# IlzeAmandaA/VAE-GP-ODE

Hardware: AMD Instinct MI355X
Metric: latent_trajectories_per_sec (higher is better)
Workload: dtype f32; 1 GPU; configs[1]: ode1 DF q=6 M=100 S=256 T=16 batch=256; step = full ELBO training step (encoder, GP draw, rk4 rollout, decoder, ELBO, backward, Adam), L=1; global_batch=256, mc_draws=1, solver=rk4 (3/8 rule), parallelism=dp1, hip_graph=True, graph_scope=whole, gp_side_stream=True, batchnorm=per-process statistics

## Files before the change

include/gpode.h:

```cpp
#ifndef GPODE_H
#define GPODE_H
#include <stddef.h>
#ifdef __cplusplus
extern "C" {
#endif

#define GPODE_KERNEL_RBF 0
#define GPODE_KERNEL_DF 1
#define GPODE_METHOD_EULER 0
#define GPODE_METHOD_RK4 1
#define GPODE_METHOD_MIDPOINT 2
#define GPODE_METHOD_DOPRI5 3

const char* gpode_version(void);
const char* gpode_last_error(void);
const char* gpode_last_launch(void);
int gpode_supported(int kernel, int Di, int Do);

int gpode_cache_sizes(int kernel, int Di, int Do, int M, int S, size_t* pack_floats, size_t* ws_floats);

int gpode_cache_build_fwd(int kernel, int Di, int Do, int M, int S,
                          const float* raw_ell, const float* raw_var, const float* Z,
                          const float* Um, const float* Us_packed,
                          const float* eps_u, const float* rff_w, const float* rff_eps, const float* rff_u,
                          float* pack, float* ws,
                          float* ell, float* var, float* omega, float* phase, float* u,
                          float* Lu, float* nu, float* u_prior, void* stream);

int gpode_rhs_fwd(int kernel, int Di, int Do, int M, int S, const float* pack,
                  const float* x, int N, float* f, int mode, void* stream);

int gpode_rollout_fwd(int kernel, int order, int method, int Di, int Do, int M, int S,
                      const float* pack, const float* z0, const float* ts, int N, int T,
                      float* zt, float* xstage, void* stream);

int gpode_rollout_bwd(int kernel, int order, int method, int Di, int Do, int M, int S,
                      const float* pack, const float* xstage, const float* gzt, const float* ts, int N, int T,
                      float* gz0, float* astage, void* stream);

int gpode_rhs_vjp(int kernel, int Di, int Do, int M, int S, const float* pack,
                  const float* x, const float* a, int R, float* gx, void* stream);

int gpode_param_grad(int kernel, int Di, int Do, int M, int S, const float* pack,
                     const float* x, const float* a, int R, float* slab, int nchunk, float* gpack, int accumulate,
                     void* stream);

int gpode_cache_bwd_sizes(int kernel, int Di, int Do, int M, int S, size_t* bws_floats);
int gpode_cache_build_bwd(int kernel, int Di, int Do, int M, int S,
                          const float* raw_ell, const float* raw_var, const float* Z, const float* eps_u,
// ... 284 lines not shown
```

vae-gp-ode_amd/_lib.py:

```python
import ctypes
import os

_HERE = os.path.dirname(os.path.abspath(__file__))
LIB_PATH = os.path.join(_HERE, 'libgpode_hip.so')

_vp = ctypes.c_void_p
_i = ctypes.c_int
_f = ctypes.c_float
_sz = ctypes.c_size_t
_sz_p = ctypes.POINTER(_sz)

SIGNATURES = {
    'gpode_version': (ctypes.c_char_p, []),
    'gpode_last_error': (ctypes.c_char_p, []),
    'gpode_last_launch': (ctypes.c_char_p, []),
    'gpode_supported': (_i, [_i, _i, _i]),
    'gpode_cache_sizes': (_i, [_i, _i, _i, _i, _i, _sz_p, _sz_p]),
    'gpode_cache_build_fwd': (_i, [_i] * 5 + [_vp] * 20),
    'gpode_cache_bwd_sizes': (_i, [_i, _i, _i, _i, _i, _sz_p]),
    'gpode_cache_build_bwd': (_i, [_i] * 5 + [_vp] * 13 + [_i, _vp]),
    'gpode_cache_bwd_prepare': (_i, [_i] * 5 + [_vp] * 2 + [_vp]),
    'gpode_cache_info': (_i, [_vp, ctypes.POINTER(_i), _vp]),
    'gpode_cache_pivots': (_i, [_vp, ctypes.POINTER(_f), _vp]),
    'gpode_set_backward_solves': (_i, [_i]),
    'gpode_kernel_matrix': (_i, [_i, _i, _i, _vp, _vp, _vp, _i, _vp, _i, _vp, _vp]),
    'gpode_conditional_ws': (_i, [_i, _i, _i, _i, _sz_p]),
    'gpode_conditional': (_i, [_i, _i, _i, _i] + [_vp] * 5 + [_i, _vp, _i] + [_vp] * 3 + [_vp]),
    'gpode_conditional_df_ws': (_i, [_i, _i, _i, _sz_p]),
    'gpode_conditional_df': (_i, [_i, _i, _i] + [_vp] * 6 + [_i] + [_vp] * 3 + [_vp]),
    'gpode_svgp_kl_fwd': (_i, [_i, _i, _vp, _vp, _vp, _vp]),
    'gpode_svgp_kl_bwd': (_i, [_i, _i] + [_vp] * 5 + [_vp]),
    'gpode_rhs_fwd': (_i, [_i] * 5 + [_vp, _vp, _i, _vp, _i, _vp]),
    'gpode_rollout_fwd': (_i, [_i] * 7 + [_vp, _vp, _vp, _i, _i, _vp, _vp, _vp]),
    'gpode_rollout_bwd': (_i, [_i] * 7 + [_vp] * 4 + [_i, _i, _vp, _vp, _vp]),
    'gpode_rhs_vjp': (_i, [_i] * 5 + [_vp, _vp, _vp, _i, _vp, _vp]),
    'gpode_rhs_jvp': (_i, [_i] * 6 + [_vp, _vp, _i, _vp, _i, _i, _vp, _vp, _i, _vp]),
    'gpode_rollout_jvp': (_i, [_i] * 8 + [_vp, _vp, _i, _vp, _i, _vp, _i, _i, _i, _i, _vp, _vp, _vp]),
    'gpode_param_grad': (_i, [_i] * 5 + [_vp, _vp, _vp, _i, _vp, _i, _vp, _i, _vp]),
    'gpode_cache_sizes_n': (_i, [_i] * 6 + [_sz_p, _sz_p]),
    'gpode_cache_build_fwd_n': (_i, [_i] * 6 + [_vp] * 20),
    'gpode_rollout_fwd_n': (_i, [_i] * 8 + [_vp, _vp, _vp, _i, _i, _vp, _vp, _vp]),
    'gpode_rollout_bwd_n': (_i, [_i] * 8 + [_vp] * 4 + [_i, _i, _vp, _vp, _vp]),
    'gpode_rollout_adaptive_fwd_n': (_i, [_i] * 8 + [_vp] * 3 + [_i, _i, _f, _f, _i] + [_vp] * 5 + [_vp]),
    'gpode_rollout_adaptive_bwd_n': (_i, [_i] * 8 + [_vp] * 5 + [_i, _i, _i, _vp, _vp, _vp]),
    'gpode_rollout_dense_fwd_n': (_i, [_i] * 8 + [_vp] * 3 + [_i, _i, _f, _f, _i] + [_vp] * 6 + [_vp]),
    'gpode_rollout_dense_bwd_n': (_i, [_i] * 8 + [_vp] * 6 + [_i, _i, _i, _vp, _vp, _vp]),
    'gpode_rollout_fwd_nz': (_i, [_i] * 8 + [_vp, _vp, _vp, _i, _i, _vp, _vp, _i, _vp]),
    'gpode_rollout_adaptive_fwd_nz': (_i, [_i] * 8 + [_vp] * 3 + [_i, _i, _f, _f, _i] + [_vp] * 5 + [_i, _vp]),
# ... 132 lines not shown
```

vae-gp-ode_amd/csrc/capi.hip:

```cpp
#include "../../include/gpode.h"
#include "gp_launch.hpp"

namespace gp {
char* error_slot() {
  static thread_local char buf[512] = {0};
  return buf;
}
const char** last_launch_slot() {
  static thread_local const char* tag = "";
  return &tag;
}
bool* force_substep_kernels() {
  static bool on = false;
  return &on;
}
}

extern "C" {

const char* gpode_version(void) { return "gpode-hip 0.1 (gfx950)"; }
const char* gpode_last_error(void) { return gp::error_slot(); }
const char* gpode_last_launch(void) { return *gp::last_launch_slot(); }
int gpode_supported(int kernel, int Di, int Do) { return gp::dims_supported(kernel, Di, Do); }

int gpode_cache_sizes(int kernel, int Di, int Do, int M, int S, size_t* pack_floats, size_t* ws_floats) {
  return gp::cache_sizes(kernel, Di, Do, M, S, pack_floats, ws_floats, 1);
}
int gpode_cache_sizes_n(int kernel, int Di, int Do, int M, int S, int ndraws, size_t* pack_floats, size_t* ws_floats) {
  return gp::cache_sizes(kernel, Di, Do, M, S, pack_floats, ws_floats, ndraws);
}

int gpode_cache_build_fwd_n(int kernel, int Di, int Do, int M, int S, int ndraws,
                            const float* raw_ell, const float* raw_var, const float* Z,
                            const float* Um, const float* Us_packed,
                            const float* eps_u, const float* rff_w, const float* rff_eps, const float* rff_u,
                            float* pack, float* ws,
                            float* ell, float* var, float* omega, float* phase, float* u,
                            float* Lu, float* nu, float* u_prior, void* stream) {
  if (!raw_ell || !raw_var || !Z || !Um || !Us_packed || !eps_u || !rff_w || !rff_eps || !rff_u || !pack || !ws)
    return gp::set_error("gpode_cache_build_fwd: null required pointer");
  return gp::cache_build_fwd(kernel, Di, Do, M, S, ndraws, raw_ell, raw_var, Z, Um, Us_packed, eps_u, rff_w, rff_eps, rff_u,
                             pack, ws, ell, var, omega, phase, u, Lu, nu, u_prior, (hipStream_t)stream);
}
int gpode_cache_build_fwd(int kernel, int Di, int Do, int M, int S,
                          const float* raw_ell, const float* raw_var, const float* Z,
                          const float* Um, const float* Us_packed,
                          const float* eps_u, const float* rff_w, const float* rff_eps, const float* rff_u,
                          float* pack, float* ws,
                          float* ell, float* var, float* omega, float* phase, float* u,
                          float* Lu, float* nu, float* u_prior, void* stream) {
  return gpode_cache_build_fwd_n(kernel, Di, Do, M, S, 1, raw_ell, raw_var, Z, Um, Us_packed, eps_u, rff_w, rff_eps, rff_u, pack, ws, ell, var,
                                 omega, phase, u, Lu, nu, u_prior, stream);
}

int gpode_cache_info(const float* ws, int* host_info, void* stream) {
// ... 867 lines not shown
```

vae-gp-ode_amd/csrc/conv_fwd_v2.hpp:

```cpp
#pragma once
#include "conv_mfma.hpp"

namespace gp {

template <class L> struct FwV2 {
  using PL = FwdPolicy<L, L::CO>;
  template <int CLS> using C = typename PL::template C<CLS>;
  static constexpr int KC = L::CI, NC = L::CO, KK = L::K * L::K, KG = KC / 4;
  static_assert(NC == 16 && L::S == 2 && PL::NCLS == 4, "one co tile, four stride-parity classes");
  static constexpr int NKS = KK * KG;
  static constexpr int NPX = C<0>::npc;
  static_assert(C<1>::npc == NPX && C<2>::npc == NPX && C<3>::npc == NPX && C<1>::nx == C<0>::nx && C<2>::nx == C<0>::nx &&
                C<3>::nx == C<0>::nx, "the classes share one q-grid");
  static constexpr int SH = L::HI, OHW = L::HO * L::HO;
  static constexpr int SRC = KC * SH * SH;
  static constexpr int PS = PL::PS, HP = PL::HP, PADL = PL::PADL, IMG = KC * PS;
  static constexpr int NCW = 4, NTHR = 64 * (NCW + 4), NLT = NTHR - 64 * NCW;
  static constexpr int TPW = 2;
  static constexpr int WIN = 16 * NCW * TPW;
  static constexpr int PF = 2;
  static constexpr int NBUF = (2 * WIN - 2) / NPX + 2;
  static constexpr int MAXS = PADL * (HP + 1);
  static constexpr int TFO = (HP * HP + 3) / 4 * 4;
  static_assert(igemm_tf_in_pad<PL>(), "the input-transform table fits the plane tails");
// ... 205 lines not shown
            }
          }
        });
      }
      __syncthreads();
    }
  }

  if constexpr (STATS) {
    float* red = s_buf + E::RED;
    float* s_sm = red + E::NSW * 2 * NC;
    const int lr = lane & 15, lk = lane >> 4;
#pragma unroll
    for (int e = 0; e < 2; ++e)
#pragma unroll
      for (int r = 0; r < 4; ++r) {
        const float a = row_allreduce16(bs[e][r]), b = row_allreduce16(bq[e][r]);
        if (lr == 0 && wave >= NCW) {
          red[((wave - NCW + NCW * e) * NC + 4 * lk + r) * 2] = a;
          red[((wave - NCW + NCW * e) * NC + 4 * lk + r) * 2 + 1] = b;
        }
      }
    __syncthreads();
    if (tid < 2 * NC) {
      float t = 0.f;
      for (int wv = 0; wv < E::NSW; ++wv) t += red[wv * 2 * NC + tid];
      s_sm[tid] = t;
    }
    __syncthreads();
    bn_sink_publish<NC, E::NTHR>(sink, s_sm);
  }
}

}
```

vae-gp-ode_amd/csrc/conv_mfma.hpp:

```cpp
#pragma once
#include <hip/hip_runtime.h>
#include <cstdint>
#include <type_traits>
#include "bn_math.hpp"
#include "bn_sink.hpp"

namespace gp {

typedef float f32x4 __attribute__((ext_vector_type(4)));

template <int N, class F> __device__ __forceinline__ void static_for(F&& f) {
  if constexpr (N > 0) {
    static_for<N - 1>(f);
    f(std::integral_constant<int, N - 1>{});
  }
}

#ifdef CONVT_PROBE
__device__ unsigned long long g_probe[8];
#define PROBE_T(v) const long long v = clock64()
#define PROBE_ADD(i, v) do { if (threadIdx.x == 0 && blockIdx.x == 0) g_probe[i] += (unsigned long long)(clock64() - (v)); } while (0)
#else
#define PROBE_T(v)
#define PROBE_ADD(i, v)
// ... 75 lines not shown
    const float* wp = sw + ((size_t)t * KC + cb + lk) * WROW + lr;
    const int ao = CG::tap_off(t) + cb * PS;
#pragma unroll
    for (int kk = 0; kk < KB; ++kk) {
#pragma unroll
      for (int c = 0; c < NCJ; ++c) bf[kk][c] = wp[4 * kk * WROW + c * 16];
#pragma unroll
      for (int g = 0; g < NG; ++g) af[kk][g] = s_img[abase[g] + ao + 4 * kk * PS];
    }
  };
  auto mma = [&](const float (&bf)[KB][NCJ], const float (&af)[KB][NG]) {
#pragma unroll
    for (int kk = 0; kk < KB; ++kk)
#pragma unroll
      for (int g = 0; g < NG; ++g)
#pragma unroll
        for (int c = 0; c < NCJ; ++c)
          acc[g][c] = __builtin_amdgcn_mfma_f32_16x16x4f32(bf[kk][c], af[kk][g], acc[g][c], 0, 0, 0);
  };
  fetch(0, bfA, afA);
  int s = 0;
  while (true) {
    if (s + 1 < nsteps) fetch(s + 1, bfB, afB);
    mma(bfA, afA);
    if (++s >= nsteps) break;
    if (s + 1 < nsteps) fetch(s + 1, bfA, afA);
    mma(bfB, afB);
    if (++s >= nsteps) break;
  }
}

extern __shared__ __attribute__((aligned(16))) float igemm_smem[];

template <class PL, int IPB, int TG, int NCJ, bool PAIR, int NTHR, bool STATS = false>
__global__ __launch_bounds__(NTHR, NTHR == 256 ? 2 : 1) void k_conv_igemm(const float* __restrict__ x, const float* __restrict__ w,
                                                      const float* __restrict__ bias, float* __restrict__ y, int B,
                                                      const float* __restrict__ in_bn, BnSink sink) {
  constexpr int KC = PL::KC, NC = PL::NC, NCS = PL::NCS, NCLS = PL::NCLS, SH = PL::SH, OH = PL::OH, HP = PL::HP, PS = PL::PS;
  constexpr int PADL = PL::PADL, WROW = PL::WROW, NWE = PL::NWE;
  static_assert(NCS % 16 == 0 && NC % NCS == 0 && KC % 4 == 0 && NTHR % 256 == 0, "MFMA tiling");
  constexpr int NW = NTHR / 64;
  constexpr int PT = NTHR;
  constexpr int NCO = NCS / 16;
  static_assert(NCO % NCJ == 0, "channel tiles per job");
  constexpr int NJ = NCO / NCJ;
  static_assert(NJ == 1 || TG == 1, "tile groups share all channel tiles");
  static_assert(!STATS || NJ == 1, "output statistics: a lane keeps the same channels in every job of a pass");
  constexpr int IMG = KC * PS;
  static_assert(IMG % 4 == 0, "float4 zero fill");
  constexpr int SRC = KC * SH * SH;
  static_assert(SRC % 4 == 0, "float4 source fetch");
  constexpr int NLD = (IPB * SRC / 4 + PT - 1) / PT;
  float* s_img = igemm_smem;
  float* s_w = igemm_smem + IPB * IMG;
  constexpr int TFO = (HP * HP + 3) / 4 * 4;
  constexpr bool TF_PAD = igemm_tf_in_pad<PL>();
  float* s_sm = s_w + PL::WSLAB + (TF_PAD ? 0 : 4 * KC);
  float4* s_tf_tail = reinterpret_cast<float4*>(s_w + PL::WSLAB);
  auto tf_slot = [&](int ch) -> float4* { return TF_PAD ? reinterpret_cast<float4*>(s_img + ch * PS + TFO) : s_tf_tail + ch; };
  const int tid = threadIdx.x, lane = tid & 63, wave = __builtin_amdgcn_readfirstlane(tid >> 6);
  const int lr = lane & 15, lk = lane >> 4;
  const int ptid = tid;
  const int ngroups = (B + IPB - 1) / IPB;
  const float4* x4 = reinterpret_cast<const float4*>(x);
  const int jw = (wave & 3) * (NW / 4) + (wave >> 2);

  PROBE_T(pt_all);
  for (int e = tid; e < IPB * IMG / 4; e += NTHR) reinterpret_cast<float4*>(s_img)[e] = float4{0.f, 0.f, 0.f, 0.f};
  if (in_bn) {
    if (TF_PAD) __syncthreads();
    for (int e = tid; e < KC; e += NTHR) *tf_slot(e) = reinterpret_cast<const float4*>(in_bn)[e];
  }
  if (STATS)
    for (int e = tid; e < 2 * NC; e += NTHR) s_sm[e] = 0.f;

  constexpr int NPASS = NC / NCS;
  const bool spread = NPASS > 1 && gridDim.x % NPASS == 0;
  const int gstride = spread ? gridDim.x / NPASS : gridDim.x;
  const int gfirst = spread ? blockIdx.x % gstride : blockIdx.x;
  for (int pass = spread ? blockIdx.x / gstride : 0; pass < (spread ? blockIdx.x / gstride + 1 : NPASS); ++pass) {
    const int n0 = pass * NCS;
    __syncthreads();
    PROBE_T(pt_w);
    for (int base = 0; base < NWE; base += NTHR * 8) {
      float v[8];
#pragma unroll
      for (int u = 0; u < 8; ++u) {
        const int e = base + tid + NTHR * u;
        v[u] = e < NWE ? w[PL::w_src(e, n0)] : 0.f;
      }
#pragma unroll
      for (int u = 0; u < 8; ++u) {
        const int e = base + tid + NTHR * u;
        if (e < NWE) s_w[PL::w_dst(e)] = v[u];
      }
    }
    PROBE_ADD(0, pt_w);

    float kshift[NCJ][4], bs[NCJ][4], bq[NCJ][4];
#pragma unroll
    for (int cc = 0; cc < NCJ; ++cc)
#pragma unroll
      for (int r = 0; r < 4; ++r) {
        kshift[cc][r] = STATS ? bn_sink_shift(sink, n0 + cc * 16 + 4 * lk + r) : 0.f;
        bs[cc][r] = bq[cc][r] = 0.f;
      }
    float4 pre[NLD];
    auto prefetch = [&](int grp) __attribute__((always_inline)) {
      const int b0 = grp * IPB;
      const int nf4 = min(IPB, B - b0) * (SRC / 4);
      const float4* src = x4 + (size_t)b0 * (SRC / 4);
#pragma unroll
      for (int i = 0; i < NLD; ++i) {
        const int f = ptid + PT * i;
        if (f < nf4) pre[i] = src[f];
      }
// ... 18 lines not shown
    };
    auto jobs = [&](const float* __restrict__ img, int b0, int nimg, int pf_grp) {
      PROBE_T(pt_rng);
      int wtot = 0;
      constexpr int NCG = PAIR ? NCLS / 2 : NCLS;
      static_for<NCG>([&](auto c) {
        constexpr int c0 = PAIR ? 2 * decltype(c)::value : decltype(c)::value;
        using G0 = typename PL::template C<c0>;
        using G1 = typename PL::template C<PAIR ? c0 + 1 : c0>;
        wtot += ((nimg * G0::npc + 15) / 16) * NJ * (G0::ntaps + (PAIR ? G1::ntaps : 0));
      });
      const int lo = (wtot * jw) / NW, hi = (wtot * (jw + 1)) / NW;
      int cbase = 0;
      PROBE_ADD(0, pt_rng);
      static_for<NCG>([&](auto c) {
        constexpr int c0 = PAIR ? 2 * decltype(c)::value : decltype(c)::value;
        using G = typename PL::template C<c0>;
        using G1 = typename PL::template C<PAIR ? c0 + 1 : c0>;
        static_assert(!PAIR || (G::npc == G1::npc && G::nx == G1::nx), "paired classes cover the same pixel grid");
        static_assert(!PAIR || (G::out_off(0) == G1::out_off(0) + 1 && G::out_off(G::npc - 1) == G1::out_off(G::npc - 1) + 1 &&
                                G1::out_off(0) % 2 == 0 && OH % 2 == 0), "paired classes write neighbouring, 8-byte aligned columns");
        constexpr int ntaps = G::ntaps + (PAIR ? G1::ntaps : 0), npc = G::npc;
        const float* swc = s_w + G::slab_taps * KC * WROW;
        const float* swc1 = s_w + G1::slab_taps * KC * WROW;
        const int mtot = nimg * npc;
        const int njobs = ((mtot + 15) / 16) * NJ;
        const int nlo = lo - cbase - ntaps / 2, nhi = hi - cbase - ntaps / 2;
        const int ub = min(njobs, nlo <= 0 ? 0 : (nlo + ntaps - 1) / ntaps), ue = min(njobs, nhi <= 0 ? 0 : (nhi + ntaps - 1) / ntaps);
        cbase += njobs * ntaps;
        for (int u0 = ub; u0 < ue; u0 += TG) {
          PROBE_T(pt_su);
          const int ng = min(TG, ue - u0);
          const int t0 = u0 / NJ, jc = u0 % NJ;
          int abase[TG], abase1[TG];
#pragma unroll
          for (int g = 0; g < TG; ++g) {
            int m = (t0 + g) * 16 + lr;
            m = (g < ng && m < mtot) ? m : 0;
            const int im = m / npc, p = m % npc;
            abase[g] = im * IMG + lk * PS + G::pix_addr(p);
            abase1[g] = im * IMG + lk * PS + G1::pix_addr(p);
          }
          f32x4 acc[TG][NCJ], acc1[TG][NCJ];
#pragma unroll
          for (int g = 0; g < TG; ++g)
#pragma unroll
            for (int cc = 0; cc < NCJ; ++cc) acc[g][cc] = acc1[g][cc] = f32x4{0.f, 0.f, 0.f, 0.f};
          float bv[NCJ][4];
#pragma unroll
          for (int cc = 0; cc < NCJ; ++cc)
#pragma unroll
            for (int r = 0; r < 4; ++r) bv[cc][r] = bias ? bias[n0 + (jc * NCJ + cc) * 16 + 4 * lk + r] : 0.f;
          PROBE_ADD(6, pt_su);
          PROBE_T(pt_mm);
          auto run = [&](auto gtag, const float* sw, const int (&ab)[TG], f32x4 (&ac)[TG][NCJ]) {
            using GG = typename decltype(gtag)::type;
            switch (ng) {
              case 1: igemm_tile_mma<GG, 1, TG, NCJ, KC, WROW, PS>(img, sw, ab, lk, lr, ac); break;
              case 2: if constexpr (TG >= 2) igemm_tile_mma<GG, 2, TG, NCJ, KC, WROW, PS>(img, sw, ab, lk, lr, ac); break;
              case 3: if constexpr (TG >= 3) igemm_tile_mma<GG, 3, TG, NCJ, KC, WROW, PS>(img, sw, ab, lk, lr, ac); break;
              default: if constexpr (TG >= 4) igemm_tile_mma<GG, 4, TG, NCJ, KC, WROW, PS>(img, sw, ab, lk, lr, ac); break;
            }
          };
          run(std::common_type<G>{}, swc + jc * NCJ * 16, abase, acc);
          if (pf_grp >= 0) { prefetch(pf_grp); pf_grp = -1; }
          if constexpr (PAIR) run(std::common_type<G1>{}, swc1 + jc * NCJ * 16, abase1, acc1);
          PROBE_ADD(3, pt_mm);
          PROBE_T(pt_st);
#pragma unroll
          for (int g = 0; g < TG; ++g) {
            const int m = (t0 + g) * 16 + lr;
            if (g < ng && m < mtot) {
              const int im = m / npc, p = m % npc;
              const int ch0 = n0 + jc * NCJ * 16 + 4 * lk;
              float* yp = y + ((size_t)(b0 + im) * NC + ch0) * (OH * OH) + (PAIR ? G1::out_off(p) : G::out_off(p));
#pragma unroll
              for (int cc = 0; cc < NCJ; ++cc)
#pragma unroll
                for (int r = 0; r < 4; ++r) {
                  const float v0 = acc[g][cc][r] + bv[cc][r];
                  if constexpr (PAIR) {
                    const float v1 = acc1[g][cc][r] + bv[cc][r];
                    *reinterpret_cast<float2*>(yp + (size_t)(cc * 16 + r) * (OH * OH)) = float2{v1, v0};
                    if (STATS) { const float d = v1 - kshift[cc][r]; bs[cc][r] += d; bq[cc][r] = fmaf(d, d, bq[cc][r]); }
                  } else {
                    yp[(size_t)(cc * 16 + r) * (OH * OH)] = v0;
                  }
                  if (STATS) { const float d = v0 - kshift[cc][r]; bs[cc][r] += d; bq[cc][r] = fmaf(d, d, bq[cc][r]); }
                }
            }
          }
          PROBE_ADD(4, pt_st);
        }
      });
      if (pf_grp >= 0) prefetch(pf_grp);
    };
    if (gfirst < ngroups) prefetch(gfirst);
    for (int grp = gfirst; grp < ngroups; grp += gstride) {
      const int b0 = grp * IPB;
      const int nimg = min(IPB, B - b0);
      PROBE_T(pt_b1);
      __syncthreads();
      PROBE_ADD(1, pt_b1);
      PROBE_T(pt_sc);
      scatter(s_img, nimg);
      __syncthreads();
      PROBE_ADD(2, pt_sc);
      PROBE_T(pt_pf);
      PROBE_ADD(7, pt_pf);
      jobs(s_img, b0, nimg, grp + gstride < ngroups ? grp + gstride : -1);
    }
    if constexpr (STATS) {
      __syncthreads();
      float* red = s_w;
#pragma unroll
      for (int cc = 0; cc < NCJ; ++cc)
#pragma unroll
        for (int r = 0; r < 4; ++r) {
          const float a = row_allreduce16(bs[cc][r]), b = row_allreduce16(bq[cc][r]);
          if (lr == 0 && wave < NW) {
            red[(wave * NCS + cc * 16 + 4 * lk + r) * 2] = a;
            red[(wave * NCS + cc * 16 + 4 * lk + r) * 2 + 1] = b;
          }
        }
      __syncthreads();
      if (tid < 2 * NCS) {
        float t = 0.f;
        for (int wv = 0; wv < NW; ++wv) t += red[wv * NCS * 2 + tid];
        s_sm[2 * n0 + tid] = t;
      }
    }
  }
  if constexpr (STATS) {
// ... 226 lines not shown
```

vae-gp-ode_amd/csrc/gp_launch.hpp:

```cpp
#pragma once
#include <cstdint>
#include <cstdlib>
#include <hip/hip_runtime.h>
#include <cstdarg>
#include <cstdio>
#include <mutex>
#include <unordered_map>

namespace gp {

char* error_slot();
const char** last_launch_slot();

inline int set_error(const char* fmt, ...) {
  va_list ap;
  va_start(ap, fmt);
  vsnprintf(error_slot(), 512, fmt, ap);
  va_end(ap);
  return 1;
}

inline int check_launch(const char* what) {
  *last_launch_slot() = what;
  hipError_t e = hipGetLastError();
  if (e != hipSuccess) return set_error("%s: launch failed: %s", what, hipGetErrorString(e));
  return 0;
}

inline bool env_flag(const char* name) {
  const char* e = getenv(name);
  return e && e[0] == '1';
}

template <class... T> inline bool aligned16(const T*... p) {
  return ((uintptr_t{0} | ... | reinterpret_cast<uintptr_t>(p)) & 15) == 0;
}

inline int set_max_lds(const void* kern, size_t bytes) {
  if (bytes <= 64 * 1024) return 0;
  static std::mutex mu;
  static std::unordered_map<const void*, size_t> done;
  std::lock_guard<std::mutex> lock(mu);
  auto it = done.find(kern);
  if (it != done.end() && it->second >= bytes) return 0;
  hipError_t e = hipFuncSetAttribute(kern, hipFuncAttributeMaxDynamicSharedMemorySize, (int)bytes);
  if (e != hipSuccess) return set_error("hipFuncSetAttribute(max dynamic LDS=%zu): %s", bytes, hipGetErrorString(e));
  done[kern] = bytes;
  return 0;
}

inline int ew_grid(size_t n) { size_t g = (n + 255) / 256; return (int)(g < 8192 ? (g ? g : 1) : 8192); }

inline int num_cus() {
  static const int n = [] {
    int dev = 0, v = 0;
    if (hipGetDevice(&dev) != hipSuccess || hipDeviceGetAttribute(&v, hipDeviceAttributeMultiprocessorCount, dev) != hipSuccess || v <= 0)
// ... 207 lines not shown
```

vae-gp-ode_amd/csrc/vae_conv_tiled.hip:

```cpp
#include <hip/hip_runtime.h>
#include <cstdlib>
#include "gp_launch.hpp"
#include "conv_layers.hpp"
#include "conv_mfma.hpp"
#include "conv_dec10_mfma.hpp"
#include "conv_dec1_mfma.hpp"
#include "conv_dec4_mfma.hpp"

namespace gp {

extern __shared__ __attribute__((aligned(16))) float tsm[];

template <class L, int IPB>
__global__ __launch_bounds__(256) void k_convT_fwd(const float* __restrict__ x, const float* __restrict__ w,
                                                    const float* __restrict__ bias, float* __restrict__ y, int B) {
  constexpr int CI = L::CI, CO = L::CO, HI = L::HI, HO = L::HO, HP = L::HP, K = L::K, S = L::S, P = L::P, PL = L::PL;
  constexpr int CPT = CO % 16 == 0 ? 16 : 8;
  static_assert(CO % CPT == 0, "8 or 16 output channels per thread");
  constexpr int NG = CO / CPT;
  constexpr int IMG = CI * HP * HP;
  float* s_img = tsm;
  float* s_w = tsm + IPB * IMG;
  const int tid = threadIdx.x;
  const int b0 = blockIdx.x * IPB;
// ... 275 lines not shown
  }
}

__global__ void k_sum_splits_t(const float* __restrict__ part, int nsplit, size_t n, float* __restrict__ out) {
  const size_t e = (size_t)blockIdx.x * blockDim.x + threadIdx.x;
  if (e >= n) return;
  float acc = 0.f;
  for (int s = 0; s < nsplit; ++s) acc += part[(size_t)s * n + e];
  out[e] = acc;
}

template <class L> static bool matches(const ConvGeom& g) {
  return g.Ci == L::CO && g.Co == L::CI && g.H == L::HO && g.Ho == L::HI && g.K == L::K && g.S == L::S && g.P == L::P;
}

static bool use_mfma() {
  static const bool valu = env_flag("GPODE_CONV_VALU");
  return !valu;
}

constexpr int kSinkMaxWg = 512;

template <class PL, int IPB, int TG, int NCJ, bool PAIR = false, int NTHR = 512, bool STATS = false>
static int launch_igemm(const float* x, const float* w, const float* bias, float* y, int B, hipStream_t st, const char* what,
                        const float* in_bn = nullptr, const BnSink* sink = nullptr) {
  constexpr size_t lds = igemm_lds_bytes<PL, IPB, STATS>();
  static_assert(lds <= (NTHR >= 512 ? 160 : 80) * 1024, "LDS budget");
  auto km = k_conv_igemm<PL, IPB, TG, NCJ, PAIR, NTHR, STATS>;
  if (set_max_lds((const void*)km, lds)) return 1;
  const int ngroups = (B + IPB - 1) / IPB;
  const int cap = num_cus() * (NTHR >= 512 ? 1 : 2);
  if (STATS && cap > kSinkMaxWg) return set_error("%s: more workgroups than the statistics scratch holds", what);
  hipLaunchKernelGGL(km, ngroups < cap ? ngroups : cap, NTHR, lds, st, x, w, bias, y, B, in_bn, STATS ? *sink : BnSink{});
  return check_launch(what);
}

template <class L, int IPB, int IPBM, int COS>
static int launch_T1(const float* x, const float* w, const float* bias, float* y, int B, hipStream_t st, const float* in_bn,
                     const BnSink* sink = nullptr) {
  if (use_mfma() && aligned16(x, w, y, in_bn)) {
    constexpr int TG = COS >= 64 ? 1 : (COS >= 32 ? 2 : 4);
    constexpr bool PAIR = L::S == 2 && (L::HO % 2 == 0) && (L::P % 2 == 1);
    if (sink) return launch_igemm<FwdPolicy<L, COS>, IPBM, TG, COS / 16, PAIR, 512, true>(x, w, bias, y, B, st, "convT_fwd_mfma_stats", in_bn, sink);
    return launch_igemm<FwdPolicy<L, COS>, IPBM, TG, COS / 16, PAIR>(x, w, bias, y, B, st, "convT_fwd_mfma", in_bn);
  }
  if (sink) return set_error("convT forward with output statistics needs the matrix-core path (16-byte aligned operands, GPODE_CONV_VALU unset)");
  if (in_bn) return set_error("convT forward with a fused BatchNorm input needs the matrix-core path (16-byte aligned operands, GPODE_CONV_VALU unset)");
  constexpr int MAXTAPS = ((L::K + L::S - 1) / L::S) * ((L::K + L::S - 1) / L::S);
  const size_t lds = sizeof(float) * ((size_t)IPB * L::CI * L::HP * L::HP + (size_t)MAXTAPS * L::CI * L::CO);
  auto kern = k_convT_fwd<L, IPB>;
  if (set_max_lds((const void*)kern, lds)) return 1;
  hipLaunchKernelGGL(kern, (B + IPB - 1) / IPB, 256, lds, st, x, w, bias, y, B);
  return check_launch("convT_fwd_tiled");
}

template <class L, int IPB, int COC>
static int launch_T2(const float* gy, const float* w, float* gx, int B, hipStream_t st) {
  const size_t lds = sizeof(float) * ((size_t)IPB * L::CO * L::GP_ * L::GP_ + (size_t)COC * L::K * L::K * L::CI);
  auto kern = k_convT_bwd_data<L, IPB, COC>;
  if (set_max_lds((const void*)kern, lds)) return 1;
  hipLaunchKernelGGL(kern, (B + IPB - 1) / IPB, 256, lds, st, gy, w, gx, B);
  return check_launch("convT_bwd_data_tiled");
}

template <class L, int WM, int WN, int WT>
static int launch_wgrad_mfma(const float* x, const float* gy, float* gw, float* scratch, int B, hipStream_t st, const float* in_bn) {
  constexpr int IPBM = 8, NTHR = WM * WN * WT * 64;
// ... 5 lines not shown
  const int ngroups = (B + IPBM - 1) / IPBM;
  const int nwg = ngroups < num_cus() ? ngroups : num_cus();
  if (in_bn) hipLaunchKernelGGL(kb, nwg, NTHR, ldsm, st, x, gy, scratch, B, in_bn);
  else hipLaunchKernelGGL(km, nwg, NTHR, ldsm, st, x, gy, scratch, B, in_bn);
  const size_t n = (size_t)L::CI * L::CO * L::K * L::K;
  if (reduce_job(RedJob{scratch, gw, nwg, (int)n, 1, L::CI / 16, L::CO / 16, L::K * L::K}, st)) return 1;
  return check_launch("convT_wgrad_mfma");
}

template <class L, int COW>
static int launch_T3(const float* x, const float* gy, float* gw, float* scratch, int B, hipStream_t st, const float* in_bn) {
  if (in_bn) return set_error("convT weight gradient with a fused BatchNorm input needs the matrix-core path (16-byte aligned operands, GPODE_CONV_VALU unset)");
  constexpr int NT = L::CI * (COW / 4), PSPLIT = 256 / NT, KK = L::K * L::K;
  size_t fl = (size_t)L::HI * L::HI * L::CI + (size_t)L::GP_ * L::GP_ * COW;
  const size_t red = PSPLIT > 1 ? (size_t)PSPLIT * NT * KK * 4 : 0;
  if (red > fl) fl = red;
  const size_t lds = sizeof(float) * fl;
  int nsplit = B < 256 ? B : 256;
  const int bps = (B + nsplit - 1) / nsplit;
  nsplit = (B + bps - 1) / bps;
  auto kern = k_convT_wgrad<L, COW>;
  if (set_max_lds((const void*)kern, lds)) return 1;
  hipLaunchKernelGGL(kern, dim3(nsplit, L::CO / COW), 256, lds, st, x, gy, scratch, B, bps);
  const size_t n = (size_t)L::CI * L::CO * KK;
  if (reduce_job(RedJob{scratch, gw, nsplit, (int)n, 0, 0, 0, 0}, st)) return 1;
  return check_launch("convT_wgrad_tiled");
}


int conv_v2_dec7_bwd_data(const float* gy, const float* w, float* gx, int B, hipStream_t st);
int conv_v2_dec4_bwd_data(const float* gy, const float* w, float* gx, int B, hipStream_t st);
int conv_v2_dec7_fwd(const float* x, const float* w, const float* bias, float* y, int B, const float* in_bn, const BnSink* sink,
                     hipStream_t st);
static bool conv_v1() {
  static const bool on = env_flag("GPODE_CONV_V1");
  return on;
}

int tiled_bwd_data(const float* gy, const float* w, const float* bias, float* gx, const ConvGeom& g, const float* in_bn, hipStream_t st,
                   const BnSink* sink) {
  if (g.H != g.W || g.Ho != g.Wo) return -1;
  const int B = g.B;
  if (sink && !(matches<Dec7>(g) || matches<Dec4>(g) ||
                (matches<Dec1>(g) && !in_bn)))
    return set_error("gpode_convT_fwd_stats: no specialisation for this geometry");
  const bool mfma = use_mfma() && aligned16(gy, w, gx, in_bn);
  if (matches<Dec7>(g)) {
    if (mfma && !conv_v1()) return conv_v2_dec7_fwd(gy, w, bias, gx, B, in_bn, sink, st);
    return launch_T1<Dec7, 3, 2, 16>(gy, w, bias, gx, B, st, in_bn, sink);
  }
  if (matches<Dec4>(g)) {
    static const int tapcols = [] { const char* e = getenv("GPODE_DEC4_TAPCOLS"); return e ? (e[0] == '1' ? 1 : 0) : -1; }();
    if ((tapcols == 1 || (tapcols < 0 && B <= 4 * num_cus())) && mfma) {
      const size_t lds = sizeof(float) * (dec4::NPI * dec4::TLD + 4 * dec4::CI + (sink ? 2 * dec4::CO * dec4::NPO : 0));
      if (set_max_lds((const void*)dec4::k_fwd<true>, lds) || set_max_lds((const void*)dec4::k_fwd<false>, lds) ||
          set_max_lds((const void*)dec4::k_fwd<true, true>, lds) || set_max_lds((const void*)dec4::k_fwd<false, true>, lds)) return 1;
      const int nwg = B < num_cus() ? B : num_cus();
      const BnSink sk = sink ? *sink : BnSink{};
      if (sink && in_bn) hipLaunchKernelGGL((dec4::k_fwd<true, true>), nwg, 512, lds, st, gy, w, bias, gx, B, in_bn, sk);
      else if (sink) hipLaunchKernelGGL((dec4::k_fwd<false, true>), nwg, 512, lds, st, gy, w, bias, gx, B, in_bn, sk);
      else if (in_bn) hipLaunchKernelGGL((dec4::k_fwd<true>), nwg, 512, lds, st, gy, w, bias, gx, B, in_bn, sk);
      else hipLaunchKernelGGL((dec4::k_fwd<false>), nwg, 512, lds, st, gy, w, bias, gx, B, in_bn, sk);
      return check_launch("dec4_fwd_tapcols");
    }
    return launch_T1<Dec4, 3, 2, 16>(gy, w, bias, gx, B, st, in_bn, sink);
  }
  if (matches<Dec1>(g)) {
    if (!in_bn && mfma) {
      const size_t lds = sizeof(float) * 2 * dec1::NPI * dec1::TLD;
      if (set_max_lds((const void*)dec1::k_fwd<false>, lds) || set_max_lds((const void*)dec1::k_fwd<true>, lds)) return 1;
      const int cap = 2 * num_cus();
      if (sink) hipLaunchKernelGGL(dec1::k_fwd<true>, B < cap ? B : cap, 256, lds, st, gy, w, bias, gx, B, *sink);
      else hipLaunchKernelGGL(dec1::k_fwd<false>, B < cap ? B : cap, 256, lds, st, gy, w, bias, gx, B, BnSink{});
      return check_launch("dec1_fwd_mfma");
    }
    if (sink) return set_error("convT forward with output statistics needs the matrix-core path (16-byte aligned operands, GPODE_CONV_VALU unset)");
    return launch_T1<Dec1, 8, 8, 64>(gy, w, bias, gx, B, st, in_bn);
  }
  if (matches<Enc3>(g) && !in_bn && B >= 96) {
    constexpr int IPB = 2;
    constexpr int MAXTAPS = ((Enc3::K + Enc3::S - 1) / Enc3::S) * ((Enc3::K + Enc3::S - 1) / Enc3::S);
    const size_t lds = sizeof(float) * ((size_t)IPB * Enc3::CI * Enc3::HP * Enc3::HP + (size_t)MAXTAPS * Enc3::CI * Enc3::CO);
    auto kern = k_convT_fwd<Enc3, IPB>;
    if (set_max_lds((const void*)kern, lds)) return 1;
    hipLaunchKernelGGL(kern, (B + IPB - 1) / IPB, 256, lds, st, gy, w, bias, gx, B);
    return check_launch("enc_conv3_bwd_data_tiled");
  }
  if (matches<Enc6>(g) && mfma) {
    if (B < 4 * num_cus()) return launch_igemm<FwdPolicy<Enc6, 16>, 2, 4, 1>(gy, w, bias, gx, B, st, "enc_conv6_bwd_data_mfma", in_bn);
    return launch_igemm<FwdPolicy<Enc6, 16>, 8, 4, 1>(gy, w, bias, gx, B, st, "enc_conv6_bwd_data_mfma", in_bn);
  }
  if (matches<Dec10>(g)) {
    if (mfma) {
      const size_t ldsm = sizeof(float) * dec10::KK * dec10::PST;
      if (set_max_lds((const void*)dec10::k_fwd<true>, ldsm) || set_max_lds((const void*)dec10::k_fwd<false>, ldsm)) return 1;
      if (in_bn) hipLaunchKernelGGL(dec10::k_fwd<true>, B < num_cus() ? B : num_cus(), 512, ldsm, st, gy, w, bias, gx, B, in_bn);
// ... 220 lines not shown
```

vae-gp-ode_amd/csrc/vae_conv_v2.hip:

```cpp
#include <hip/hip_runtime.h>
#include <cstdint>
#include "gp_launch.hpp"
#include "conv_layers.hpp"
#include "conv_bwd_v2.hpp"
#include "conv_fwd_v2.hpp"

namespace gp {

template <class L> static int launch_bwd_data_v2(const float* gy, const float* w, float* gx, int B, hipStream_t st, const char* what) {
  using E = BdV2<L>;
  constexpr size_t lds = E::lds_bytes();
  static_assert(lds <= 160 * 1024, "LDS budget");
  auto km = k_conv_bwd_data_v2<L>;
  if (set_max_lds((const void*)km, lds)) return 1;
  hipLaunchKernelGGL(km, B < num_cus() ? B : num_cus(), E::NTHR, lds, st, gy, w, gx, B);
  return check_launch(what);
}

int conv_v2_dec7_bwd_data(const float* gy, const float* w, float* gx, int B, hipStream_t st) {
  return launch_bwd_data_v2<Dec7>(gy, w, gx, B, st, "conv_v2_dec7_bwd_data");
}

int conv_v2_dec4_bwd_data(const float* gy, const float* w, float* gx, int B, hipStream_t st) {
  return launch_bwd_data_v2<Dec4>(gy, w, gx, B, st, "conv_v2_dec4_bwd_data");
}

template <class L, bool HAS_BN, bool STATS>
static int launch_fwd_v2(const float* x, const float* w, const float* bias, float* y, int B, const float* in_bn, const BnSink* sink,
                         hipStream_t st, const char* what) {
  using E = FwV2<L>;
  constexpr size_t lds = E::lds_bytes(STATS);
  static_assert(lds + (STATS ? sizeof(float) * (E::NTHR + 1) : 0) <= 160 * 1024, "LDS budget (with bn_sink_publish's static arrays)");
  auto km = k_conv_fwd_v2<L, HAS_BN, STATS>;
  if (set_max_lds((const void*)km, lds)) return 1;
  if (STATS && num_cus() > 512) return set_error("%s: more workgroups than the statistics scratch holds", what);
  const int nwork = STATS ? (B + E::IPG - 1) / E::IPG : B;
  hipLaunchKernelGGL(km, nwork < num_cus() ? nwork : num_cus(), E::NTHR, lds, st, x, w, bias, y, B, in_bn, STATS ? *sink : BnSink{});
  return check_launch(what);
}

int conv_v2_dec7_fwd(const float* x, const float* w, const float* bias, float* y, int B, const float* in_bn, const BnSink* sink,
                     hipStream_t st) {
  if (in_bn && sink) return launch_fwd_v2<Dec7, true, true>(x, w, bias, y, B, in_bn, sink, st, "conv_v2_dec7_fwd_bn_stats");
  if (sink) return launch_fwd_v2<Dec7, false, true>(x, w, bias, y, B, in_bn, sink, st, "conv_v2_dec7_fwd_stats");
  if (in_bn) return launch_fwd_v2<Dec7, true, false>(x, w, bias, y, B, in_bn, sink, st, "conv_v2_dec7_fwd_bn");
  return launch_fwd_v2<Dec7, false, false>(x, w, bias, y, B, in_bn, sink, st, "conv_v2_dec7_fwd");
}

}
```

Baseline: 110,200 trajectories/s.

## Add warp-specialized MFMA forward kernel for Dec4 transposed conv with stats read-back

Result: no change. 109,600 trajectories/s (-0.5%).

```diff
diff --git a/include/gpode.h b/include/gpode.h
--- a/include/gpode.h
+++ b/include/gpode.h
@@ -15,6 +15,7 @@
 const char* gpode_version(void);
 const char* gpode_last_error(void);
 const char* gpode_last_launch(void);
+const char* gpode_last_launch_engine(void);
 int gpode_supported(int kernel, int Di, int Do);
 
 int gpode_cache_sizes(int kernel, int Di, int Do, int M, int S, size_t* pack_floats, size_t* ws_floats);
diff --git a/vae-gp-ode_amd/_lib.py b/vae-gp-ode_amd/_lib.py
--- a/vae-gp-ode_amd/_lib.py
+++ b/vae-gp-ode_amd/_lib.py
@@ -14,6 +14,7 @@
     'gpode_version': (ctypes.c_char_p, []),
     'gpode_last_error': (ctypes.c_char_p, []),
     'gpode_last_launch': (ctypes.c_char_p, []),
+    'gpode_last_launch_engine': (ctypes.c_char_p, []),
     'gpode_supported': (_i, [_i, _i, _i]),
     'gpode_cache_sizes': (_i, [_i, _i, _i, _i, _i, _sz_p, _sz_p]),
     'gpode_cache_build_fwd': (_i, [_i] * 5 + [_vp] * 20),
diff --git a/vae-gp-ode_amd/csrc/capi.hip b/vae-gp-ode_amd/csrc/capi.hip
--- a/vae-gp-ode_amd/csrc/capi.hip
+++ b/vae-gp-ode_amd/csrc/capi.hip
@@ -10,6 +10,10 @@
   static thread_local const char* tag = "";
   return &tag;
 }
+const char** last_engine_slot() {
+  static thread_local const char* engine = "";
+  return &engine;
+}
 bool* force_substep_kernels() {
   static bool on = false;
   return &on;
@@ -21,6 +25,7 @@
 const char* gpode_version(void) { return "gpode-hip 0.1 (gfx950)"; }
 const char* gpode_last_error(void) { return gp::error_slot(); }
 const char* gpode_last_launch(void) { return *gp::last_launch_slot(); }
+const char* gpode_last_launch_engine(void) { return *gp::last_engine_slot(); }
 int gpode_supported(int kernel, int Di, int Do) { return gp::dims_supported(kernel, Di, Do); }
 
 int gpode_cache_sizes(int kernel, int Di, int Do, int M, int S, size_t* pack_floats, size_t* ws_floats) {
diff --git a/vae-gp-ode_amd/csrc/conv_fwd_v2.hpp b/vae-gp-ode_amd/csrc/conv_fwd_v2.hpp
--- a/vae-gp-ode_amd/csrc/conv_fwd_v2.hpp
+++ b/vae-gp-ode_amd/csrc/conv_fwd_v2.hpp
@@ -261,4 +261,170 @@
   }
 }
 
+template <class L> struct FwV2P {
+  using PL = FwdPolicy<L, 16>;
+  template <int CLS> using C = typename PL::template C<CLS>;
+  static constexpr int KC = L::CI, NC = L::CO, KK = L::K * L::K, KG = KC / 4, NCT = NC / 16;
+  static_assert(L::S == 2 && PL::NCLS == 4 && NC % 16 == 0 && KC % 4 == 0, "four stride-parity classes, whole MFMA tiles");
+  static constexpr int SH = L::HI, SQ = SH * SH, OHW = L::HO * L::HO;
+  static constexpr int SRC = KC * SQ;
+  static constexpr int PS = PL::PS, HP = PL::HP, PADL = PL::PADL, IMG = KC * PS;
+  static constexpr int NCW = 4, NTHR = 64 * (NCW + 4), NLT = NTHR - 64 * NCW;
+  static constexpr int TSPLIT = NCW / NCT;
+  static constexpr int TPW = 2;
+  static constexpr int WIN = 16 * TSPLIT * TPW;
+  static constexpr int PF = 2;
+  static constexpr int NPMIN = C<0>::npc;
+  static_assert(C<1>::npc >= NPMIN && C<2>::npc >= NPMIN && C<3>::npc >= NPMIN && C<3>::npc < 256, "ring sized for class 0; position in 8 bits");
+  static constexpr int NBUF = (2 * WIN - 2) / NPMIN + 2;
+  static constexpr int MAXW = C<0>::ntaps * KG;
+  static_assert(C<1>::ntaps <= C<0>::ntaps && C<2>::ntaps <= C<0>::ntaps && C<3>::ntaps <= C<0>::ntaps && MAXW <= 160, "weights of a phase in registers");
+  static constexpr int MAXS = PADL * (HP + 1);
+  static constexpr int TFO = (HP * HP + 3) / 4 * 4;
+  static_assert(igemm_tf_in_pad<PL>(), "the input-transform table fits the plane tails");
+  static_assert(NCW % NCT == 0 && TPW * (PF + 1) <= 15, "consumers split the co tiles evenly; LDS reads in flight within what lgkmcnt counts");
+  static constexpr int NSUB = NLT / SQ, NLD = (KG + NSUB - 1) / NSUB;
+  static_assert(SRC % 4 == 0 && NSUB >= 1, "float4 source, producer offset table");
+  static_assert(4 * (MAXS + (KG - 1) * 4 * PS) < 65536, "operand offsets fit the ds_read immediate");
+  static constexpr int CST = NBUF * IMG;
+  static constexpr size_t lds_bytes() { return sizeof(float) * ((size_t)CST + NC); }
+};
+
+template <class E, class G>
+__device__ __forceinline__ void fwv2p_tiles(const float* __restrict__ s_buf, const int (&base)[E::TPW], const float (&wr)[G::ntaps * E::KG],
+                                            f32x4 (&acc)[E::TPW]) {
+  constexpr int N = G::ntaps * E::KG;
+  float bf[E::PF + 1][E::TPW];
+  auto fetch = [&](auto sc) {
+    constexpr int S = decltype(sc)::value;
+    const int off = E::MAXS + G::tap_off(S / E::KG) + (S % E::KG) * 4 * E::PS;
+#pragma unroll
+    for (int t = 0; t < E::TPW; ++t) bf[S % (E::PF + 1)][t] = s_buf[base[t] + off];
+  };
+#pragma unroll
+  for (int t = 0; t < E::TPW; ++t) acc[t] = f32x4{0.f, 0.f, 0.f, 0.f};
+  static_for<E::PF>([&](auto sc) { fetch(sc); });
+  static_for<N>([&](auto sc) {
+    constexpr int S = decltype(sc)::value;
+    if constexpr (S + E::PF < N) fetch(std::integral_constant<int, S + E::PF>{});
+    __builtin_amdgcn_sched_barrier(0);
+#pragma unroll
+    for (int t = 0; t < E::TPW; ++t) acc[t] = __builtin_amdgcn_mfma_f32_16x16x4f32(wr[S], bf[S % (E::PF + 1)][t], acc[t], 0, 0, 0);
+    __builtin_amdgcn_sched_barrier(0);
+  });
 }
+
+template <class L, bool HAS_BN>
+__global__ __launch_bounds__(FwV2P<L>::NTHR) void k_conv_fwd_v2p(const float* __restrict__ x, const float* __restrict__ w,
+                                                                 const float* __restrict__ bias, float* __restrict__ y, int B,
+                                                                 const float* __restrict__ in_bn) {
+  using E = FwV2P<L>;
+  constexpr int KC = E::KC, NC = E::NC, KK = E::KK, KG = E::KG, IMG = E::IMG, PS = E::PS, HP = E::HP, WIN = E::WIN, SQ = E::SQ;
+  constexpr int SH = E::SH, PADL = E::PADL, NBUF = E::NBUF, TPW = E::TPW, NCW = E::NCW, OHW = E::OHW, TSPLIT = E::TSPLIT;
+  float* s_buf = igemm_smem;
+  const int tid = threadIdx.x, lane = tid & 63, wave = __builtin_amdgcn_readfirstlane(tid >> 6);
+  const int bx = blockIdx.x, ngx = gridDim.x;
+  const int nit = bx < B ? (B - 1 - bx) / ngx + 1 : 0;
+
+  for (int e = tid; e < NBUF * IMG / 4; e += E::NTHR) reinterpret_cast<float4*>(s_buf)[e] = float4{0.f, 0.f, 0.f, 0.f};
+  if (tid < NC) s_buf[E::CST + tid] = bias ? bias[tid] : 0.f;
+  __syncthreads();
+  if constexpr (HAS_BN) {
+    for (int e = tid; e < KC; e += E::NTHR) *reinterpret_cast<float4*>(s_buf + e * PS + E::TFO) = reinterpret_cast<const float4*>(in_bn)[e];
+    __syncthreads();
+  }
+
+  if (wave >= NCW) {
+    __builtin_amdgcn_s_setprio(3);
+    const int lt = tid - 64 * NCW;
+    constexpr int N4 = E::SRC / 4;
+    const int sub = lt / SQ, q4 = lt % SQ;
+    int otab[4], opl[4];
+#pragma unroll
+    for (int k = 0; k < 4; ++k) {
+      const int e = 4 * q4 + k, pl = e / SQ, q = e % SQ;
+      opl[k] = pl * PS;
+      otab[k] = pl * PS + (q / SH + PADL) * HP + q % SH + PADL;
+    }
+    auto stage = [&](int j) __attribute__((always_inline)) {
+      const float4* src = reinterpret_cast<const float4*>(x) + (size_t)(bx + j * ngx) * N4;
+      float* buf = s_buf + (j % NBUF) * IMG;
+      if (sub < E::NSUB) {
+        float4 v[E::NLD];
+#pragma unroll
+        for (int i = 0; i < E::NLD; ++i) v[i] = src[min(sub + E::NSUB * i, KG - 1) * SQ + q4];
+#pragma unroll
+        for (int i = 0; i < E::NLD; ++i) {
+          const int g = sub + E::NSUB * i;
+          if (g < KG) {
+            float* d = buf + 4 * g * PS;
+            float e[4] = {v[i].x, v[i].y, v[i].z, v[i].w};
+            if constexpr (HAS_BN) {
+#pragma unroll
+              for (int k = 0; k < 4; ++k) e[k] = bn_relu(e[k], *reinterpret_cast<const float4*>(s_buf + 4 * g * PS + opl[k] + E::TFO));
+            }
+            d[otab[0]] = e[0]; d[otab[1]] = e[1]; d[otab[2]] = e[2]; d[otab[3]] = e[3];
+          }
+        }
+      }
+    };
+    static_for<4>([&](auto cc) {
+      constexpr int npc = E::template C<decltype(cc)::value>::npc;
+      const int npx = nit * npc, nwin = (npx + WIN - 1) / WIN;
+      auto last_img = [&](int i) { return min(nit - 1, (i * WIN + WIN - 1) / npc); };
+      int staged = -1;
+      if (nit > 0)
+        for (; staged < last_img(0); ) stage(++staged);
+      __syncthreads();
+      for (int i = 0; i < nwin; ++i) {
+        if (i + 1 < nwin)
+          for (const int j1 = last_img(i + 1); staged < j1; ) stage(++staged);
+        __syncthreads();
+      }
+    });
+    __builtin_amdgcn_s_setprio(0);
+  } else {
+    const int lr = lane & 15, lk = lane >> 4, u = wave / TSPLIT, h = wave % TSPLIT;
+    static_for<4>([&](auto cc) {
+      using G = typename E::template C<decltype(cc)::value>;
+      constexpr int NS = G::ntaps * KG, npc = G::npc;
+      const int npx = nit * npc, nwin = (npx + WIN - 1) / WIN;
+      float wr[NS];
+#pragma unroll
+      for (int s = 0; s < NS; ++s) {
+        const int t = s / KG, ky = G::py + L::S * (t / G::ntx), kx = G::px + L::S * (t % G::ntx);
+        wr[s] = w[((size_t)(4 * (s % KG) + lk) * NC + 16 * u + lr) * KK + ky * L::K + kx];
+      }
+      __syncthreads();
+      for (int i = 0; i < nwin; ++i) {
+        const int t0 = i * WIN + 16 * h;
+        if (t0 < npx) {
+          int jp[TPW], base[TPW];
+#pragma unroll
+          for (int t = 0; t < TPW; ++t) {
+            const int m = min(t0 + 16 * TSPLIT * t + lr, npx - 1);
+            const int j = m / npc, p = m - j * npc;
+            jp[t] = j << 8 | p;
+            base[t] = (j % NBUF) * IMG + lk * PS - E::MAXS + G::pix_addr(p);
+          }
+          f32x4 acc[TPW];
+          fwv2p_tiles<E, G>(s_buf, base, wr, acc);
+          const float4 b4 = *reinterpret_cast<const float4*>(s_buf + E::CST + 16 * u + 4 * lk);
+          const float bv[4] = {b4.x, b4.y, b4.z, b4.w};
+#pragma unroll
+          for (int t = 0; t < TPW; ++t) {
+            if (t0 + 16 * TSPLIT * t + lr < npx) {
+              const int j = jp[t] >> 8;
+              float* yp = y + ((size_t)(bx + j * ngx) * NC + 16 * u + 4 * lk) * OHW + G::out_off(jp[t] & 255);
+#pragma unroll
+              for (int r = 0; r < 4; ++r) yp[(size_t)r * OHW] = acc[t][r] + bv[r];
+            }
+          }
+        }
+        __syncthreads();
+      }
+    });
+  }
+}
+
+}
diff --git a/vae-gp-ode_amd/csrc/conv_mfma.hpp b/vae-gp-ode_amd/csrc/conv_mfma.hpp
--- a/vae-gp-ode_amd/csrc/conv_mfma.hpp
+++ b/vae-gp-ode_amd/csrc/conv_mfma.hpp
@@ -131,6 +131,10 @@
 
 extern __shared__ __attribute__((aligned(16))) float igemm_smem[];
 
+template <class P> struct StatsReadback : P { static constexpr bool READBACK = true; };
+template <class PL, class = void> struct igemm_readback : std::false_type {};
+template <class PL> struct igemm_readback<PL, std::enable_if_t<PL::READBACK>> : std::true_type {};
+
 template <class PL, int IPB, int TG, int NCJ, bool PAIR, int NTHR, bool STATS = false>
 __global__ __launch_bounds__(NTHR, NTHR == 256 ? 2 : 1) void k_conv_igemm(const float* __restrict__ x, const float* __restrict__ w,
                                                       const float* __restrict__ bias, float* __restrict__ y, int B,
@@ -145,6 +149,8 @@
   constexpr int NJ = NCO / NCJ;
   static_assert(NJ == 1 || TG == 1, "tile groups share all channel tiles");
   static_assert(!STATS || NJ == 1, "output statistics: a lane keeps the same channels in every job of a pass");
+  constexpr bool RB = igemm_readback<PL>::value;
+  static_assert(!RB || (STATS && !PAIR), "the read-back walk is the unpaired statistics walk");
   constexpr int IMG = KC * PS;
   static_assert(IMG % 4 == 0, "float4 zero fill");
   constexpr int SRC = KC * SH * SH;
@@ -165,10 +171,12 @@
   const int jw = (wave & 3) * (NW / 4) + (wave >> 2);
 
   PROBE_T(pt_all);
-  for (int e = tid; e < IPB * IMG / 4; e += NTHR) reinterpret_cast<float4*>(s_img)[e] = float4{0.f, 0.f, 0.f, 0.f};
-  if (in_bn) {
-    if (TF_PAD) __syncthreads();
-    for (int e = tid; e < KC; e += NTHR) *tf_slot(e) = reinterpret_cast<const float4*>(in_bn)[e];
+  if constexpr (!RB) {
+    for (int e = tid; e < IPB * IMG / 4; e += NTHR) reinterpret_cast<float4*>(s_img)[e] = float4{0.f, 0.f, 0.f, 0.f};
+    if (in_bn) {
+      if (TF_PAD) __syncthreads();
+      for (int e = tid; e < KC; e += NTHR) *tf_slot(e) = reinterpret_cast<const float4*>(in_bn)[e];
+    }
   }
   if (STATS)
     for (int e = tid; e < 2 * NC; e += NTHR) s_sm[e] = 0.f;
@@ -181,6 +189,7 @@
     const int n0 = pass * NCS;
     __syncthreads();
     PROBE_T(pt_w);
+    if constexpr (!RB)
     for (int base = 0; base < NWE; base += NTHR * 8) {
       float v[8];
 #pragma unroll
@@ -265,6 +274,28 @@
           PROBE_T(pt_su);
           const int ng = min(TG, ue - u0);
           const int t0 = u0 / NJ, jc = u0 % NJ;
+          if constexpr (RB) {
+            float yv[TG][NCJ][4];
+#pragma unroll
+            for (int g = 0; g < TG; ++g) {
+              const int m = min((t0 + g) * 16 + lr, mtot - 1), im = m / npc, p = m % npc;
+              const float* yp = y + ((size_t)(b0 + im) * NC + n0 + jc * NCJ * 16 + 4 * lk) * (OH * OH) + G::out_off(p);
+#pragma unroll
+              for (int cc = 0; cc < NCJ; ++cc)
+#pragma unroll
+                for (int r = 0; r < 4; ++r) yv[g][cc][r] = yp[(size_t)(cc * 16 + r) * (OH * OH)];
+            }
+#pragma unroll
+            for (int g = 0; g < TG; ++g) {
+              if (g < ng && (t0 + g) * 16 + lr < mtot) {
+#pragma unroll
+                for (int cc = 0; cc < NCJ; ++cc)
+#pragma unroll
+                  for (int r = 0; r < 4; ++r) { const float d = yv[g][cc][r] - kshift[cc][r]; bs[cc][r] += d; bq[cc][r] = fmaf(d, d, bq[cc][r]); }
+              }
+            }
+            continue;
+          }
           int abase[TG], abase1[TG];
 #pragma unroll
           for (int g = 0; g < TG; ++g) {
@@ -328,10 +359,14 @@
       });
       if (pf_grp >= 0) prefetch(pf_grp);
     };
-    if (gfirst < ngroups) prefetch(gfirst);
+    if (!RB && gfirst < ngroups) prefetch(gfirst);
     for (int grp = gfirst; grp < ngroups; grp += gstride) {
       const int b0 = grp * IPB;
       const int nimg = min(IPB, B - b0);
+      if constexpr (RB) {
+        jobs(s_img, b0, nimg, -1);
+        continue;
+      }
       PROBE_T(pt_b1);
       __syncthreads();
       PROBE_ADD(1, pt_b1);
diff --git a/vae-gp-ode_amd/csrc/gp_launch.hpp b/vae-gp-ode_amd/csrc/gp_launch.hpp
--- a/vae-gp-ode_amd/csrc/gp_launch.hpp
+++ b/vae-gp-ode_amd/csrc/gp_launch.hpp
@@ -11,6 +11,7 @@
 
 char* error_slot();
 const char** last_launch_slot();
+const char** last_engine_slot();
 
 inline int set_error(const char* fmt, ...) {
   va_list ap;
@@ -20,8 +21,9 @@
   return 1;
 }
 
-inline int check_launch(const char* what) {
+inline int check_launch(const char* what, const char* engine = "") {
   *last_launch_slot() = what;
+  *last_engine_slot() = engine;
   hipError_t e = hipGetLastError();
   if (e != hipSuccess) return set_error("%s: launch failed: %s", what, hipGetErrorString(e));
   return 0;
diff --git a/vae-gp-ode_amd/csrc/vae_conv_tiled.hip b/vae-gp-ode_amd/csrc/vae_conv_tiled.hip
--- a/vae-gp-ode_amd/csrc/vae_conv_tiled.hip
+++ b/vae-gp-ode_amd/csrc/vae_conv_tiled.hip
@@ -331,7 +331,19 @@
   const int cap = num_cus() * (NTHR >= 512 ? 1 : 2);
   if (STATS && cap > kSinkMaxWg) return set_error("%s: more workgroups than the statistics scratch holds", what);
   hipLaunchKernelGGL(km, ngroups < cap ? ngroups : cap, NTHR, lds, st, x, w, bias, y, B, in_bn, STATS ? *sink : BnSink{});
-  return check_launch(what);
+  return check_launch(what, "v1");
+}
+
+template <class PL, int IPB, int TG, int NCJ>
+static int launch_igemm_stats_readback(float* y, int B, hipStream_t st, const char* what, const char* engine, const BnSink* sink) {
+  constexpr size_t lds = igemm_lds_bytes<PL, IPB, true>();
+  static_assert(lds <= 160 * 1024, "LDS budget");
+  auto km = k_conv_igemm<StatsReadback<PL>, IPB, TG, NCJ, false, 512, true>;
+  if (set_max_lds((const void*)km, lds)) return 1;
+  const int ngroups = (B + IPB - 1) / IPB;
+  if (num_cus() > kSinkMaxWg) return set_error("%s: more workgroups than the statistics scratch holds", what);
+  hipLaunchKernelGGL(km, ngroups < num_cus() ? ngroups : num_cus(), 512, lds, st, nullptr, nullptr, nullptr, y, B, nullptr, *sink);
+  return check_launch(what, engine);
 }
 
 template <class L, int IPB, int IPBM, int COS>
@@ -403,6 +415,8 @@
 int conv_v2_dec4_bwd_data(const float* gy, const float* w, float* gx, int B, hipStream_t st);
 int conv_v2_dec7_fwd(const float* x, const float* w, const float* bias, float* y, int B, const float* in_bn, const BnSink* sink,
                      hipStream_t st);
+int conv_v2_dec4_fwd(const float* x, const float* w, const float* bias, float* y, int B, const float* in_bn, hipStream_t st,
+                     const char* what);
 static bool conv_v1() {
   static const bool on = env_flag("GPODE_CONV_V1");
   return on;
@@ -433,6 +447,11 @@
       else if (in_bn) hipLaunchKernelGGL((dec4::k_fwd<true>), nwg, 512, lds, st, gy, w, bias, gx, B, in_bn, sk);
       else hipLaunchKernelGGL((dec4::k_fwd<false>), nwg, 512, lds, st, gy, w, bias, gx, B, in_bn, sk);
       return check_launch("dec4_fwd_tapcols");
+    }
+    if (mfma && !conv_v1()) {
+      if (conv_v2_dec4_fwd(gy, w, bias, gx, B, in_bn, st, "convT_fwd_mfma")) return 1;
+      if (!sink) return 0;
+      return launch_igemm_stats_readback<FwdPolicy<Dec4, 16>, 2, 4, 1>(gx, B, st, "convT_fwd_mfma_stats", "v2", sink);
     }
     return launch_T1<Dec4, 3, 2, 16>(gy, w, bias, gx, B, st, in_bn, sink);
   }
diff --git a/vae-gp-ode_amd/csrc/vae_conv_v2.hip b/vae-gp-ode_amd/csrc/vae_conv_v2.hip
--- a/vae-gp-ode_amd/csrc/vae_conv_v2.hip
+++ b/vae-gp-ode_amd/csrc/vae_conv_v2.hip
@@ -14,7 +14,7 @@
   auto km = k_conv_bwd_data_v2<L>;
   if (set_max_lds((const void*)km, lds)) return 1;
   hipLaunchKernelGGL(km, B < num_cus() ? B : num_cus(), E::NTHR, lds, st, gy, w, gx, B);
-  return check_launch(what);
+  return check_launch(what, "v2");
 }
 
 int conv_v2_dec7_bwd_data(const float* gy, const float* w, float* gx, int B, hipStream_t st) {
@@ -36,7 +36,7 @@
   if (STATS && num_cus() > 512) return set_error("%s: more workgroups than the statistics scratch holds", what);
   const int nwork = STATS ? (B + E::IPG - 1) / E::IPG : B;
   hipLaunchKernelGGL(km, nwork < num_cus() ? nwork : num_cus(), E::NTHR, lds, st, x, w, bias, y, B, in_bn, STATS ? *sink : BnSink{});
-  return check_launch(what);
+  return check_launch(what, "v2");
 }
 
 int conv_v2_dec7_fwd(const float* x, const float* w, const float* bias, float* y, int B, const float* in_bn, const BnSink* sink,
@@ -47,4 +47,18 @@
   return launch_fwd_v2<Dec7, false, false>(x, w, bias, y, B, in_bn, sink, st, "conv_v2_dec7_fwd");
 }
 
+int conv_v2_dec4_fwd(const float* x, const float* w, const float* bias, float* y, int B, const float* in_bn, hipStream_t st,
+                     const char* what) {
+  using E = FwV2P<Dec4>;
+  constexpr size_t lds = E::lds_bytes();
+  static_assert(lds <= 160 * 1024, "LDS budget");
+  auto kb = k_conv_fwd_v2p<Dec4, true>;
+  auto kn = k_conv_fwd_v2p<Dec4, false>;
+  if (set_max_lds((const void*)kb, lds) || set_max_lds((const void*)kn, lds)) return 1;
+  const int nwg = B < num_cus() ? B : num_cus();
+  if (in_bn) hipLaunchKernelGGL(kb, nwg, E::NTHR, lds, st, x, w, bias, y, B, in_bn);
+  else hipLaunchKernelGGL(kn, nwg, E::NTHR, lds, st, x, w, bias, y, B, in_bn);
+  return check_launch(what, "v2");
 }
+
+}
```
